# showlab/DiffSim

Measured on AMD Instinct MI355X. Metric: image-pairs/sec at 512px, SD1.5 up_blocks[0] t=600, higher is better.
Workload: dtype bf16

## Files before the change

### diffsim_amd/csrc/gemm.hip

```cpp
#include "common.h"

#include <algorithm>
#include <type_traits>

namespace dsim {

#ifdef DSIM_DEVTOOLS
int g_force_bm = 0;
int g_gemm_persistent = 1;
int g_gemm_exp = 0;
int g_gemm_skinny = 1;
unsigned long long* g_gemm_stamps = nullptr;
#endif
void gemm_tile_choice(const GemmArgs& a, int* bm, int* bn) {
    const bool geglu = a.epi == EPI_GEGLU;
    if (geglu && a.geglu_blk == 16) {
        const long tiles = (long)((a.M + 255) / 256) * (a.N / 320);
        const bool big = g_force_bm ? g_force_bm == 256 : tiles >= 256;
        *bm = big ? 256 : 128;
        *bn = big ? 320 : 160;
        return;
    }
#ifdef DSIM_DEVTOOLS
    const bool n320 = !geglu && a.N % 320 == 0 && !(g_gemm_exp & 4096), n256 = a.N % 256 == 0;
#else
    const bool n320 = !geglu && a.N % 320 == 0, n256 = a.N % 256 == 0;
#endif
    {
        const int c320 = (a.N + 319) / 320, c256 = (a.N + 255) / 256, tm = (a.M + 255) / 256, cus = cu_count();
#ifdef DSIM_DEVTOOLS
        const bool allow = !(g_gemm_exp & 16384) && !(g_gemm_exp & 4096);
#else
        const bool allow = true;
#endif
        const bool act_only = a.act == 1 && !a.gate && a.epi != EPI_RESIDUAL;
        const long r320 = ((long)tm * c320 + cus - 1) / cus, r256 = ((long)tm * c256 + cus - 1) / cus;
        if (allow && !geglu && a.mode == GEMM_LINEAR && !n320 && (act_only || (!a.act && !a.gate)) && (long)tm * c320 >= cus &&
            (long)c320 * 320 * 20 <= (long)a.N * 21 && r320 * 320 * 19 <= r256 * 256 * 20 && g_force_bm != 128) {
            *bm = 256; *bn = 320;
            return;
        }
    }
    bool n192 = !geglu && a.mode == GEMM_LINEAR && !n320 && !n256 && a.N % 192 == 0;
    if (n192 && (long)((a.N + 255) / 256) * 256 * 20 <= (long)a.N * 21 && (long)((a.M + 255) / 256) * ((a.N + 255) / 256) >= 256) {
        *bm = g_force_bm == 128 ? 128 : 256;
        *bn = g_force_bm == 128 ? 128 : 256;
        return;
    }
    const bool n128 = !geglu && a.mode == GEMM_CONV3 && a.N == 128;
    int want256 = 0;
    if (n128) {
        const long tiles = (long)((a.M + 255) / 256);
        if (tiles >= 256 && g_force_bm != 128) { *bm = 256; *bn = 128; return; }
    }
    if (n320 || n256 || n192) {
        const int bnb = n320 ? 320 : (n256 ? 256 : 192);
        const long tiles = (long)((a.M + 255) / 256) * (a.N / bnb);
        want256 = tiles >= 256;
    }
    if (a.force_big) want256 = (n320 || n256 || n192);
    if (g_force_bm == 128) want256 = 0;
    if (g_force_bm == 256) want256 = (n320 || n256 || n192);
    if (want256) { *bm = 256; *bn = n320 ? 320 : (n256 ? 256 : 192); return; }
    *bm = 128;
    *bn = (a.N % 160 == 0 && !geglu) ? 160 : 128;
#ifdef DSIM_DEVTOOLS
    const bool allow80 = !(g_gemm_exp & 2048);
#else
    const bool allow80 = true;
#endif
    if (allow80 && *bn == 160 && (long)((a.M + 127) / 128) * (a.N / 160) <= cu_count()) *bn = 80;
}

void gemm_launch_tile(const GemmArgs& a, int dtype, int* bm, int* bn) {
    gemm_tile_choice(a, bm, bn);
    const bool slow = a.act != 0 || a.gate != nullptr;
    const bool act_only = a.act == 1 && !a.gate && a.epi != EPI_RESIDUAL;
    if (*bm == 256 && *bn == 128 && dtype != DSIM_F32 && a.mode == GEMM_CONV3 && !a.bias2 && g_force_bm != 256) {
        const long hw = (long)a.Hout * a.Wout;
        if (hw >= 512L * 256 && !(hw & (hw - 1)) && a.Wout > 0 && !(a.Wout & (a.Wout - 1)) && a.M % hw == 0) *bm = 512;
    }
    if (*bm == 512) return;
    bool big = *bm == 256 && dtype != DSIM_F32;
    if (big && slow && *bn == 320 && !act_only) big = false;
    if (!big) {
        const bool n160 = *bn == 160 || (*bn == 320 && !slow) || (a.epi == EPI_GEGLU && a.geglu_blk == 16);
        const bool n80 = *bn == 80 && dtype != DSIM_F32 && !slow;
        *bm = 128;
        *bn = slow ? 128 : (n80 ? 80 : ((n160 || *bn == 80) ? 160 : 128));
    }
}

namespace {

#if defined(DSIM_DEVTOOLS) && defined(DSIM_STAMPS)
#define STAMP(t) do { __builtin_amdgcn_sched_barrier(0); asm volatile("s_memtime %0\n\ts_waitcnt lgkmcnt(0)" : "=s"(t) :: "memory"); __builtin_amdgcn_sched_barrier(0); } while (0)
#define STAMP_DECL unsigned long long st_[7] = {0, 0, 0, 0, 0, 0, 0}, sa_[6] = {0, 0, 0, 0, 0, 0}
#define STAMP_ACC(i) sa_[i] += st_[(i) + 1] - st_[i]
#else
#define STAMP(t) do { } while (0)
#define STAMP_DECL do { } while (0)
#define STAMP_ACC(i) do { } while (0)
#endif

template <typename T> struct Traits;
template <> struct Traits<h16> {
    static constexpr int BK = 64;
    static constexpr int VEC = 8;
};
template <> struct Traits<float> {
    static constexpr int BK = 32;
    static constexpr int VEC = 4;
};

template <typename T> struct Vec16T;
template <> struct Vec16T<h16> { typedef h16x8 type; };
template <> struct Vec16T<float> { typedef f32x4 type; };

__device__ __forceinline__ void load_frag(h16x8& f, const char* p) { f = *reinterpret_cast<const h16x8*>(p); }
__device__ __forceinline__ void load_frag(f32x4& f, const char* p) { f = *reinterpret_cast<const f32x4*>(p); }
__device__ __forceinline__ void mma(const h16x8& a, const h16x8& b, f32x4& c) {
    c = H16_MFMA_16x16x32(a, b, c, 0, 0, 0);
}
__device__ __forceinline__ void mma(const f32x4& a, const f32x4& b, f32x4& c) {
#pragma unroll
    for (int e = 0; e < 4; ++e) c = __builtin_amdgcn_mfma_f32_16x16x4f32(a[e], b[e], c, 0, 0, 0);
}
template <typename T> struct FragOf { typedef h16x8 type; };
template <> struct FragOf<float> { typedef f32x4 type; };

__device__ __forceinline__ float erf_as(float x) {
    const float ax = fabsf(x);
    const float t = __builtin_amdgcn_rcpf(fmaf(0.3275911f, ax, 1.0f));
    float pl = fmaf(1.061405429f, t, -1.453152027f);
    pl = fmaf(pl, t, 1.421413741f);
    pl = fmaf(pl, t, -0.284496736f);
    pl = fmaf(pl, t, 0.254829592f);
    pl *= t;
    const float e = __builtin_amdgcn_exp2f(-ax * ax * 1.4426950408889634f);
    const float r = fmaf(-pl, e, 1.0f);
    return copysignf(r, x);
}
__device__ __forceinline__ float gelu_erf(float x) { return 0.5f * x * (1.0f + erf_as(x * 0.70710678118654752f)); }

template <typename T, int BM, int BN, bool GEGLU, int WM, int WN>
constexpr int gemm_epi_bytes() {
    return WM * WN * 16 * ((GEGLU ? BN / WN / 2 : BN / WN) * (int)sizeof(T) + 16);
}
template <typename T, int BM, int BN, bool GEGLU, int WM, int WN>
constexpr int gemm_spare_bytes() {
    const int stage = (BM + BN) * 128, epi = gemm_epi_bytes<T, BM, BN, GEGLU, WM, WN>();
    return epi > stage ? ((epi - stage + 1023) / 1024) * 1024 : 0;
}
template <typename T, int BM, int BN, bool GEGLU, int WM, int WN>
constexpr int gemm_lds_bytes() {
    return 2 * (BM + BN) * 128 + gemm_spare_bytes<T, BM, BN, GEGLU, WM, WN>() +
           (BM >= 512 ? 0 : (sizeof(T) == 2 ? 2 * WM * WN * 1024 : 2 * BN * 4));
}

enum { EK_PLAIN = 0, EK_RES = 1, EK_SLOW = 2, EK_ACT = 3,
       EK_PLAIN_GN = 4, EK_RES_GN = 5 };
template <typename T, int BM, int BN, int MODE, bool GEGLU, int WM, int WN, int EKT>
__global__ __launch_bounds__(WM * WN * 64, 2) void gemm_kernel(const GemmArgs p, const int tilesN, const int ntiles, const int tilesM,
                                                               const int gn) {
    constexpr int NW = WM * WN;
    constexpr bool GNS = EKT >= EK_PLAIN_GN;
    constexpr int EK = GNS ? EKT - EK_PLAIN_GN : EKT;
    constexpr bool CONV = MODE != GEMM_LINEAR;
    constexpr bool P2 = MODE == GEMM_CONV3P;
    constexpr int BK = Traits<T>::BK;
    constexpr int VEC = Traits<T>::VEC;
    constexpr int TM = BM / (WM * 16), TN = BN / (WN * 16);
    constexpr int PS = TM >= 4 ? 2 : (TN % 5 == 0 ? 5 : 4);
    constexpr int NP = TN / PS;
    static_assert(TN % PS == 0 && (GEGLU ? TN % 2 == 0 : true), "wave tile");
    constexpr bool G16 = GEGLU && TN % 4 != 0;
    constexpr int WBN = BN / WN;
    constexpr int NA = BM / (NW * 8);
    constexpr int NBP = BN / 8;
    constexpr int NB = (NBP + NW - 1) / NW;
    constexpr int A_BYTES = BM * 128, B_BYTES = BN * 128, STAGE = A_BYTES + B_BYTES;
    constexpr int SPARE = gemm_spare_bytes<T, BM, BN, GEGLU, WM, WN>();
    typedef typename FragOf<T>::type Frag;
    extern __shared__ __attribute__((aligned(16))) char smem[];

    const int tid = threadIdx.x, lane = tid & 63, wave = tid >> 6;
    const int lrow = lane >> 3;
    const int wrow = wave * 8 + lrow;
    const unsigned celb = ((lane & 7) ^ ((wrow >> 1) & 7)) * 16;
    constexpr unsigned OOB = 0x80000000u;

    const __amdgpu_buffer_rsrc_t rA0 = __builtin_amdgcn_make_buffer_rsrc((void*)p.A0, 0, (int)p.a0_bytes, 0x00020000);
    const __amdgpu_buffer_rsrc_t rA1 = __builtin_amdgcn_make_buffer_rsrc((void*)(p.A1 ? p.A1 : p.A0), 0, (int)p.a1_bytes, 0x00020000);
    const __amdgpu_buffer_rsrc_t rW = __builtin_amdgcn_make_buffer_rsrc((void*)p.W, 0, (int)p.w_bytes, 0x00020000);
#ifdef DSIM_DEVTOOLS
    const __amdgpu_buffer_rsrc_t rO = __builtin_amdgcn_make_buffer_rsrc(p.out, 0, (p.exp & 32) ? 0 : (int)p.out_bytes, 0x00020000);
    const __amdgpu_buffer_rsrc_t rR = __builtin_amdgcn_make_buffer_rsrc((void*)(p.residual ? p.residual : p.out), 0, (p.exp & 16) ? 0 : (int)p.out_bytes, 0x00020000);
#else
    const __amdgpu_buffer_rsrc_t rO = __builtin_amdgcn_make_buffer_rsrc(p.out, 0, (int)p.out_bytes, 0x00020000);
    const __amdgpu_buffer_rsrc_t rR = __builtin_amdgcn_make_buffer_rsrc((void*)(p.residual ? p.residual : p.out), 0, (int)p.out_bytes, 0x00020000);
#endif

    int m0 = 0, n0 = 0;
    int a_iy0[NA], a_ix0[NA];
    unsigned a_base[NA], a_voff[NA];
    unsigned b_voff[NB];
    const int Hv = p.Hin << p.ups, Wv = p.Win << p.ups;
    auto setup = [&](int vb) {
        const int xcd = vb & 7, q = ntiles >> 3, r = ntiles & 7, slot = vb >> 3;
        const int bid = (xcd < r ? xcd * (q + 1) : r * (q + 1) + (xcd - r) * q) + slot;
        const int band = bid / (gn * tilesM), rem = bid - band * (gn * tilesM);
        const int bw = min(gn, tilesN - band * gn);
        const int mt = rem / bw;
        m0 = mt * BM;
        n0 = (band * gn + (rem - mt * bw)) * BN;
#pragma unroll
        for (int i = 0; i < NA; ++i) {
            const int m = m0 + i * (NW * 8) + wrow;
            if (CONV) {
                int b, oy, ox;
                if constexpr (P2) {
                    b = m >> p.lhw;
                    const int rem = m & ((1 << p.lhw) - 1);
                    oy = rem >> p.lwo; ox = rem & ((1 << p.lwo) - 1);
                } else {
                    const int hw = p.Hout * p.Wout;
                    b = m / hw;
                    const int rem = m - b * hw;
                    oy = rem / p.Wout; ox = rem - oy * p.Wout;
                }
                a_iy0[i] = (m < p.M) ? oy * p.stride - p.pad : -(1 << 20);
                a_ix0[i] = ox * p.stride - p.pad;
                a_base[i] = (unsigned)b * (unsigned)(p.Hin * p.Win);
                a_voff[i] = OOB;
            } else {
                a_iy0[i] = a_ix0[i] = 0;
                a_base[i] = (m < p.M) ? (unsigned)m : OOB;
                a_voff[i] = (m < p.M) ? (unsigned)m * (unsigned)p.C0 * (unsigned)sizeof(T) + celb : OOB;
            }
        }
        const unsigned wofs = (!CONV && p.wb_rows) ? (unsigned)(m0 / p.wb_rows) * p.wb_stride : 0u;
#pragma unroll
        for (int i = 0; i < NB; ++i) {
            const int n = n0 + i * (NW * 8) + wrow;
            b_voff[i] = (n < p.N) ? wofs + (unsigned)n * (unsigned)p.K * (unsigned)sizeof(T) + celb : OOB;
        }
    };
    const int wave_u = __builtin_amdgcn_readfirstlane(wave);
    const bool b_tail = (NBP % NW == 0) || wave_u < (NBP % NW);
    const int wm_u = wave_u / WN, wn_u = wave_u - wm_u * WN;
    constexpr bool BDMA = sizeof(T) == 2 && BM < 512;
    static_assert(!BDMA || (BN / WN) * 4 <= 1024, "bias slot");
    const __amdgpu_buffer_rsrc_t rBias = __builtin_amdgcn_make_buffer_rsrc((void*)(p.bias ? (const void*)p.bias : p.W), 0, p.bias ? p.N * 4 : 0, 0x00020000);
    auto bias_dma = [&](int par) {
        if (BDMA && !p.bias2)
            __builtin_amdgcn_raw_ptr_buffer_load_lds(rBias, (__attribute__((address_space(3))) void*)(smem + 2 * STAGE + SPARE + (par * NW + wave_u) * 1024), 16,
                                                     (int)((unsigned)(n0 + wn_u * (BN / WN)) * 4u + (unsigned)lane * 16u), 0, 0, 0);
    };

    auto derive = [&](int t) {
        const int k0 = t * BK;
        if (CONV) {
            const int tap = k0 / p.C0;
            if (k0 == tap * p.C0) {
                const int ky = tap / 3, kx = tap - ky * 3;
#pragma unroll
                for (int i = 0; i < NA; ++i) {
                    const int iy = a_iy0[i] + ky, ix = a_ix0[i] + kx;
                    const bool ok = (unsigned)iy < (unsigned)Hv && (unsigned)ix < (unsigned)Wv;
                    const unsigned pix = a_base[i] + (unsigned)((iy >> p.ups) * p.Win + (ix >> p.ups));
                    a_voff[i] = ok ? pix * (unsigned)p.C0 * (unsigned)sizeof(T) + celb : OOB;
                }
            }
        } else if (k0 == p.C0) {
#pragma unroll
            for (int i = 0; i < NA; ++i)
                a_voff[i] = a_base[i] != OOB ? a_base[i] * (unsigned)p.C1 * (unsigned)sizeof(T) + celb : OOB;
        }
    };
#define DMAW wave_u
    auto issue = [&](int t, int buf) {
        char* sa = smem + (buf ? STAGE + SPARE : 0);
        char* sb = sa + A_BYTES;
        const int k0 = t * BK;
        int soff;
        bool second = false;
        if (CONV) {
            const int tap = k0 / p.C0;
            soff = (k0 - tap * p.C0) * (int)sizeof(T);
        } else {
            second = k0 >= p.C0;
            soff = (second ? k0 - p.C0 : k0) * (int)sizeof(T);
        }
#ifdef DSIM_DEVTOOLS
        const bool skipA = CONV && (((p.exp & 64) && (k0 / p.C0) % 3 != 0) || ((p.exp & 128) && t > 0));
#else
        constexpr bool skipA = false;
#endif
        if (!skipA) {
#pragma unroll
        for (int i = 0; i < NA; ++i) {
            auto lds = (__attribute__((address_space(3))) void*)(sa + (i * NW + DMAW) * 1024);
            if (second) __builtin_amdgcn_raw_ptr_buffer_load_lds(rA1, lds, 16, (int)a_voff[i], soff, 0, 0);
            else        __builtin_amdgcn_raw_ptr_buffer_load_lds(rA0, lds, 16, (int)a_voff[i], soff, 0, 0);
        }
        }
        const int soffw = k0 * (int)sizeof(T);
#pragma unroll
        for (int i = 0; i < NB; ++i)
            if (i + 1 < NB || b_tail)
                __builtin_amdgcn_raw_ptr_buffer_load_lds(rW, (__attribute__((address_space(3))) void*)(sb + (i * NW + DMAW) * 1024),
                                                         16, (int)b_voff[i], soffw, 0, 0);
    };
    auto stage = [&](int t, int buf) { derive(t); issue(t, buf); };

    f32x4 acc[TM][TN];
    const int nk = p.K / BK;
    const int wm = wave / WN, wn = wave - wm * WN;
    const int quad = lane >> 4;
    const int foff0 = (lane & 15) * 128 + ((quad ^ ((lane >> 1) & 7)) << 4);

    Frag xf[2][TM], wf[2][PS];
    auto load_x = [&](int buf, int step, int set) {
        const char* sa = smem + (buf ? STAGE + SPARE : 0) + wm * (BM / WM) * 128 + (foff0 ^ (step << 6));
#pragma unroll
        for (int i = 0; i < TM; ++i) load_frag(xf[set][i], sa + i * 16 * 128);
    };
    auto load_w = [&](int buf, int q, int set) {
        const int step = q / NP, j0 = (q - step * NP) * PS;
        const char* sb = smem + (buf ? STAGE + SPARE : 0) + A_BYTES + (wn * WBN + j0 * 16) * 128 + (foff0 ^ (step << 6));
#pragma unroll
        for (int j = 0; j < PS; ++j) load_frag(wf[set][j], sb + j * 16 * 128);
    };
    auto mma_piece = [&](int q) {
        const int step = q / NP, j0 = (q - step * NP) * PS;
#pragma unroll
        for (int j = 0; j < PS; ++j)
#pragma unroll
            for (int i = 0; i < TM; ++i) mma(wf[q & 1][j], xf[step][i], acc[i][j0 + j]);
    };

    constexpr int ES = sizeof(T);
    constexpr int OUTW = GEGLU ? WBN / 2 : WBN;
    constexpr int RSO = OUTW * ES + 16;
    constexpr int CPR = OUTW * ES / 16;
    const int Nout = GEGLU ? (p.N >> 1) : (p.out_split ? p.out_split : p.N);
    typedef typename Vec16T<T>::type V16;
    typedef unsigned u32x4 __attribute__((ext_vector_type(4)));
    constexpr int NIT = (16 * CPR + 63) / 64;
    constexpr bool SLOW = EK == EK_SLOW;
    constexpr bool ACT = EK == EK_ACT;
    constexpr bool BIAS_INIT = !CONV || BM >= 512;
    const bool has_res = EK == EK_RES || (SLOW && p.epi == EPI_RESIDUAL);

    STAMP_DECL;
#ifdef DSIM_DEVTOOLS
    if ((p.exp >> 8) & 15) {
        if ((blockIdx.x >> 3) & 1) {
            const int n = ((p.exp >> 8) & 15) * 2;
            for (int i = 0; i < n; ++i) __builtin_amdgcn_s_sleep(127);
        }
    }
#endif
    int vb = blockIdx.x;
    int tile_par = 0;
    int b0 = 0;
    setup(vb);
    bias_dma(0);
    stage(0, 0);
    bool first = true;
    constexpr int NST = TM * NIT;
    static_assert(NST <= 60, "counted vmcnt");
    while (true) {
        STAMP(st_[0]);
        float* const bias_lds = BDMA ? reinterpret_cast<float*>(smem + 2 * STAGE + SPARE + (tile_par * NW + wave_u) * 1024) - wn_u * WBN
                                     : reinterpret_cast<float*>(smem + 2 * STAGE + SPARE) + (tile_par ? BN : 0);
        const bool bias_in_lds = !BIAS_INIT && (BDMA ? !p.bias2 : (p.bias && !p.bias2));
        if (!BDMA && bias_in_lds && tid < BN / 4) {
            const int n = n0 + tid * 4;
            f32x4 b4 = {0.f, 0.f, 0.f, 0.f};
            if (p.bias && n < p.N) b4 = *reinterpret_cast<const f32x4*>(p.bias + n);
            *reinterpret_cast<f32x4*>(bias_lds + tid * 4) = b4;
        }
        if constexpr (BDMA) {
#ifdef DSIM_DEVTOOLS
            if (first || (p.exp & 32768)) asm volatile("s_waitcnt vmcnt(0)" ::: "memory");
#else
            if (first) asm volatile("s_waitcnt vmcnt(0)" ::: "memory");
#endif
            else asm volatile("s_waitcnt vmcnt(%0)" :: "n"(NST) : "memory");
            first = false;
        }
        if (BIAS_INIT && p.bias) {
            int ilane = lane;
            asm volatile("" : "+v"(ilane));
            const int iquad = ilane >> 4, il15 = ilane & 15;
            bool odd[TM];
#pragma unroll
            for (int i = 0; i < TM; ++i)
                odd[i] = p.bias2 && (((m0 + wm * (BM / WM) + i * 16 + il15) / p.rows_per_batch) & 1);
#pragma unroll
            for (int j = 0; j < TN; ++j) {
                const int nb = n0 + wn * WBN + j * 16 + 4 * iquad;
                f32x4 b4 = {0.f, 0.f, 0.f, 0.f}, c4 = {0.f, 0.f, 0.f, 0.f};
                if (BDMA && !p.bias2) {
                    b4 = *reinterpret_cast<const f32x4*>(bias_lds + (nb - n0));
                } else if (nb < p.N) {
                    b4 = *reinterpret_cast<const f32x4*>(p.bias + nb);
                    if (p.bias2) c4 = *reinterpret_cast<const f32x4*>(p.bias2 + nb);
                }
#pragma unroll
                for (int i = 0; i < TM; ++i)
#pragma unroll
                    for (int e = 0; e < 4; ++e) acc[i][j][e] = odd[i] ? c4[e] : b4[e];
            }
        } else {
#pragma unroll
            for (int i = 0; i < TM; ++i)
#pragma unroll
                for (int j = 0; j < TN; ++j)
#pragma unroll
                    for (int r = 0; r < 4; ++r) acc[i][j][r] = 0.0f;
        }
        STAMP(st_[1]);
        if constexpr (BDMA) {
            asm volatile("s_waitcnt lgkmcnt(0)" ::: "memory");
            __builtin_amdgcn_s_barrier();
            asm volatile("" ::: "memory");
        } else {
            asm volatile("s_waitcnt vmcnt(0)" ::: "memory");
            __syncthreads();
        }
        STAMP(st_[2]);
        load_x(b0, 0, 0);
        load_w(b0, 0, 0);
        for (int t = 0; t < nk; ++t) {
            const int cur = b0 ^ (t & 1);
            if (t + 1 < nk) stage(t + 1, cur ^ 1);
#pragma unroll
            for (int q = 0; q + 1 < 2 * NP; ++q) {
                if (q == 0) load_x(cur, 1, 1);
                load_w(cur, q + 1, (q + 1) & 1);
                __builtin_amdgcn_sched_barrier(0);
                mma_piece(q);
                __builtin_amdgcn_sched_barrier(0);
            }
#ifdef DSIM_DEVTOOLS
            if (!(p.exp & 512)) asm volatile("s_waitcnt vmcnt(0)" ::: "memory");
            if (!(p.exp & 256)) __syncthreads(); else asm volatile("s_waitcnt lgkmcnt(0)" ::: "memory");
#else
            asm volatile("s_waitcnt vmcnt(0)" ::: "memory");
            __syncthreads();
#endif
            if (t + 1 < nk) { load_x(cur ^ 1, 0, 0); load_w(cur ^ 1, 0, 0); }
            __builtin_amdgcn_sched_barrier(0);
            mma_piece(2 * NP - 1);
            __builtin_amdgcn_sched_barrier(0);
        }
        STAMP(st_[3]);
        const int xbuf = b0 ^ ((nk - 1) & 1);
        const int em0 = m0, en0 = n0;
        const int nvb = vb + (int)gridDim.x;
        const bool more = nvb < ntiles;
        if (more) {
            setup(nvb);
            bias_dma(tile_par ^ 1);
            stage(0, xbuf ^ 1);
        }
        STAMP(st_[4]);
        int elane = lane;
        asm volatile("" : "+v"(elane));
        const int el15 = elane & 15, equad = elane >> 4;
        char* const wst = smem + (xbuf ? STAGE : 0) + wave * (16 * RSO);
        const int nw0 = en0 + wn * WBN;
        int osel = 0;
        if (!GEGLU && EK == EK_PLAIN && MODE == GEMM_LINEAR && p.out_split) osel = __builtin_amdgcn_readfirstlane(en0 / p.out_split);
        const __amdgpu_buffer_rsrc_t rOt = (!GEGLU && EK == EK_PLAIN && MODE == GEMM_LINEAR)
            ? __builtin_amdgcn_make_buffer_rsrc((char*)p.out + (size_t)osel * p.out_split_stride, 0, (int)p.out_bytes, 0x00020000) : rO;
        const int nout0 = (GEGLU ? (nw0 >> 1) : nw0) - osel * p.out_split;
        const int mw0 = em0 + wm * (BM / WM);
        const int mw0_u = em0 + wm_u * (BM / WM);
        const int nout0_u = (GEGLU ? ((en0 + wn_u * WBN) >> 1) : (en0 + wn_u * WBN)) - osel * p.out_split;
        const unsigned sbase = (unsigned)(mw0_u * p.ldo + nout0_u) * (unsigned)ES;
        const unsigned sslab = 16u * (unsigned)p.ldo * (unsigned)ES;
        unsigned lp[NIT];
        int lrd[NIT];
        {
            int plane = lane;
            asm volatile("" : "+v"(plane));
#pragma unroll
            for (int it = 0; it < NIT; ++it) {
                const int idx = plane + it * 64;
                const int row = idx / CPR, c = idx - row * CPR;
                lp[it] = (idx < 16 * CPR && nout0 + c * VEC < Nout) ? (unsigned)(row * p.ldo + c * VEC) * (unsigned)ES : OOB;
                lrd[it] = (row < 16 ? row : 15) * RSO + c * 16;
            }
        }
        auto piece_v = [&](int, int, int it) -> unsigned { return lp[it]; };
        auto piece_s = [&](int i) -> int { return (int)(sbase + (unsigned)i * sslab); };
        auto store_v = [&](int i, int it) -> unsigned { return lp[it] == OOB ? OOB : lp[it] + sbase + (unsigned)i * sslab; };
        constexpr int PF0 = TM > 1 ? (NIT + 1) / 2 : (NIT < 10 ? NIT : 10);
        u32x4 rres[TM][NIT];
        auto prefetch = [&](int i, int it0, int it1) {
#pragma unroll
            for (int it = 0; it < NIT; ++it)
                if (it >= it0 && it < it1)
                    rres[i][it] = __builtin_amdgcn_raw_buffer_load_b128(rR, (int)piece_v(elane, i, it), piece_s(i), 0);
        };
        constexpr bool RES16 = EK == EK_RES && sizeof(T) == 2 && !GEGLU && CONV;
        float gq[4] = {0.f, 0.f, 0.f, 0.f};
        auto gn_acc = [&](const V16& o) {
            if constexpr (GNS) {
#pragma unroll
                for (int e = 0; e < VEC; ++e) {
                    const float f = (float)o[e];
                    gq[e >> 2] += f;
                    gq[2 + (e >> 2)] = fmaf(f, f, gq[2 + (e >> 2)]);
                }
            }
        };
        if constexpr (RES16) {
            h16x4 pk[TM][TN];
            constexpr int HP = TM >= 2 ? TM / 2 : 1;
#pragma unroll
            for (int h0 = 0; h0 < TM; h0 += HP) {
                int boff = (wn * WBN + 4 * equad) * 4;
                asm volatile("" : "+v"(boff));
#pragma unroll
                for (int j = 0; j < TN; ++j) {
                    f32x4 b4 = {0.f, 0.f, 0.f, 0.f};
                    if constexpr (!BIAS_INIT) b4 = *reinterpret_cast<const f32x4*>(reinterpret_cast<const char*>(bias_lds) + boff + j * 64);
#pragma unroll
                    for (int i = h0; i < h0 + HP; ++i) {
                        typedef float f32x2 __attribute__((ext_vector_type(2)));
                        float v[4];
#pragma unroll
                        for (int e = 0; e < 4; ++e) v[e] = BIAS_INIT ? acc[i][j][e] : acc[i][j][e] + b4[e];
                        const h16x2 lo = __builtin_convertvector((f32x2){v[0], v[1]}, h16x2), hi = __builtin_convertvector((f32x2){v[2], v[3]}, h16x2);
                        pk[i][j] = (h16x4){lo[0], lo[1], hi[0], hi[1]};
                        asm volatile("" : "+v"(pk[i][j]) :: "memory");
                    }
                }
                __builtin_amdgcn_sched_barrier(0);
#pragma unroll
                for (int i = h0; i < h0 + HP; ++i) prefetch(i, 0, NIT);
                __builtin_amdgcn_sched_barrier(0);
            }
#pragma unroll
            for (int i = 0; i < TM; ++i) {
#pragma unroll
                for (int j = 0; j < TN; ++j)
                    *reinterpret_cast<h16x4*>(wst + el15 * RSO + (j * 16 + 4 * equad) * ES) = pk[i][j];
                int slane = lane;
                asm volatile("" : "+v"(slane));
#pragma unroll
                for (int it = 0; it < NIT; ++it) {
                    const V16 t = *reinterpret_cast<const V16*>(wst + lrd[it]);
                    const V16 r = __builtin_bit_cast(V16, rres[i][it]);
                    typedef float f32x2 __attribute__((ext_vector_type(2)));
                    V16 o16;
#pragma unroll
                    for (int e = 0; e < VEC; e += 2) {
                        const h16x2 pr = __builtin_convertvector((f32x2){(float)t[e] + (float)r[e], (float)t[e + 1] + (float)r[e + 1]}, h16x2);
                        o16[e] = pr[0]; o16[e + 1] = pr[1];
                    }
                    if (lp[it] != OOB) gn_acc(o16);
                    __builtin_amdgcn_raw_buffer_store_b128(__builtin_bit_cast(u32x4, o16), rO, (int)store_v(i, it), 0, 0);
                }
            }
        } else {
#pragma unroll
        for (int i = 0; i < TM; ++i) {
            __builtin_amdgcn_sched_barrier(0);
            if (has_res) prefetch(i, 0, PF0);
            __builtin_amdgcn_sched_barrier(0);
            const int slab_half_div = (SLOW && p.gate2) ? (mw0 + i * 16) / p.rows_per_batch : 0;
            const bool odd_half = !BIAS_INIT && p.bias2 && (((mw0 + i * 16 + el15) / p.rows_per_batch) & 1);
#pragma unroll
            for (int j = 0; j < TN; ++j) {
                if (GEGLU && (j & (G16 ? 1 : 2))) continue;
                float v[4];
                if (GEGLU) {
                    constexpr int JG = G16 ? 1 : 2;
#pragma unroll
                    for (int e = 0; e < 4; ++e) v[e] = acc[i][j][e] * (sizeof(T) == 2 ? gelu_fast(acc[i][j + JG][e]) : gelu_erf(acc[i][j + JG][e]));
                } else if (BIAS_INIT) {
#pragma unroll
                    for (int e = 0; e < 4; ++e) v[e] = acc[i][j][e];
                } else {
                    const int nb = nw0 + j * 16 + 4 * equad;
                    f32x4 b4 = {0.f, 0.f, 0.f, 0.f};
                    if (bias_in_lds) {
                        b4 = *reinterpret_cast<const f32x4*>(bias_lds + (nb - en0));
                    } else if (p.bias && nb < p.N) {
                        b4 = *reinterpret_cast<const f32x4*>(p.bias + nb);
                        if (p.bias2) {
                            const f32x4 c4 = *reinterpret_cast<const f32x4*>(p.bias2 + nb);
#pragma unroll
                            for (int e = 0; e < 4; ++e) b4[e] = odd_half ? c4[e] : b4[e];
                        }
                    }
#pragma unroll
                    for (int e = 0; e < 4; ++e) v[e] = acc[i][j][e] + b4[e];
                }
                const int col = (GEGLU ? (G16 ? (j >> 1) : ((j >> 2) * 2 + (j & 1))) : j) * 16 + 4 * equad;
                char* dst = wst + el15 * RSO + col * ES;
                if constexpr (sizeof(T) == 2) {
                    typedef float f32x2 __attribute__((ext_vector_type(2)));
                    const h16x2 lo = __builtin_convertvector((f32x2){v[0], v[1]}, h16x2), hi = __builtin_convertvector((f32x2){v[2], v[3]}, h16x2);
                    const h16x4 pk = {lo[0], lo[1], hi[0], hi[1]};
                    *reinterpret_cast<h16x4*>(dst) = pk;
                } else {
                    f32x4 pk = {v[0], v[1], v[2], v[3]};
                    *reinterpret_cast<f32x4*>(dst) = pk;
                }
            }
            if (has_res && PF0 < NIT) prefetch(i, PF0, NIT);
            int slane = lane;
            asm volatile("" : "+v"(slane));
#pragma unroll
            for (int it = 0; it < NIT; ++it) {
                const V16 t = *reinterpret_cast<const V16*>(wst + lrd[it]);
                if (!SLOW && !ACT && !has_res) {
                    if (lp[it] != OOB) gn_acc(t);
                    __builtin_amdgcn_raw_buffer_store_b128(__builtin_bit_cast(u32x4, t), rOt, (int)store_v(i, it), 0, 0);
                    continue;
                }
                float v[VEC];
#pragma unroll
                for (int e = 0; e < VEC; ++e) v[e] = (float)t[e];
                if (ACT || (SLOW && p.act == 1)) {
#pragma unroll
                    for (int e = 0; e < VEC; ++e) {
                        const float x = v[e];
                        const float t = x * fmaf(-0.10294324f, x * x, -2.3022082f);
                        v[e] = x * __builtin_amdgcn_rcpf(1.0f + __builtin_amdgcn_exp2f(t));
                    }
                }
                if (SLOW && p.gate) {
                    const int idx = slane + it * 64;
                    const int row = idx / CPR, c = idx - row * CPR, rrow = row < 16 ? row : 15;
                    const int m = mw0 + i * 16 + rrow, ncol = nout0 + c * VEC;
                    if (ncol < Nout) {
                        const bool odd = p.gate2 && ((((p.rows_per_batch & 15) == 0 ? slab_half_div : m / p.rows_per_batch)) & 1);
                        const float* gsel = odd ? p.gate2 : p.gate;
#pragma unroll
                        for (int e = 0; e < VEC; e += 4) {
                            const f32x4 g4 = *reinterpret_cast<const f32x4*>(gsel + ncol + e);
#pragma unroll
                            for (int f = 0; f < 4; ++f) v[e + f] *= g4[f];
                        }
                    }
                }
                if (has_res) {
                    const V16 r = __builtin_bit_cast(V16, rres[i][it]);
#pragma unroll
                    for (int e = 0; e < VEC; ++e) v[e] += (float)r[e];
                }
                V16 o16;
                if constexpr (sizeof(T) == 2) {
                    typedef float f32x2 __attribute__((ext_vector_type(2)));
#pragma unroll
                    for (int e = 0; e < VEC; e += 2) {
                        const h16x2 pr = __builtin_convertvector((f32x2){v[e], v[e + 1]}, h16x2);
                        o16[e] = pr[0]; o16[e + 1] = pr[1];
                    }
                } else {
#pragma unroll
                    for (int e = 0; e < VEC; ++e) o16[e] = (T)v[e];
                }
                __builtin_amdgcn_raw_buffer_store_b128(__builtin_bit_cast(u32x4, o16), rO, (int)store_v(i, it), 0, 0);
            }
        }
        }
        if constexpr (GNS) {
            static_assert(sizeof(T) == 2 && CONV && !GEGLU && 64 % CPR == 0 && (CPR == 8 || CPR == 16), "epilogue statistics: 64- or 128-column wave tiles");
#pragma unroll
            for (int off = 32; off >= CPR; off >>= 1)
#pragma unroll
                for (int k = 0; k < 4; ++k) gq[k] += __shfl_xor(gq[k], off, 64);
            int glane = lane;
            asm volatile("" : "+v"(glane));
            if (glane < CPR) {
                const int img = em0 / p.gn_hw, chunk = ((em0 - img * p.gn_hw) / BM) * WM + wm_u;
                const int quads = p.N >> 2, q0 = ((en0 + wn_u * WBN) >> 2) + glane * 2;
                float* o = p.gn_part + (((size_t)img * (p.gn_hw / (BM / WM)) + chunk) * quads + q0) * 2;
                *reinterpret_cast<f32x4*>(o) = (f32x4){gq[0], gq[2], gq[1], gq[3]};
            }
        }
        STAMP(st_[5]);
        STAMP_ACC(0); STAMP_ACC(1); STAMP_ACC(2); STAMP_ACC(3); STAMP_ACC(4);
        if (!more) break;
        vb = nvb;
        tile_par ^= 1;
        asm volatile("" : "+s"(vb));
        setup(vb);
        derive(0);
        b0 = xbuf ^ 1;
        STAMP(st_[6]);
        STAMP_ACC(5);
    }
#if defined(DSIM_DEVTOOLS) && defined(DSIM_STAMPS)
    if (p.stamps && lane == 0)
        for (int i = 0; i < 6; ++i) atomicAdd(p.stamps + i, sa_[i]);
    if (p.stamps && tid == 0) atomicAdd(p.stamps + 6, 1ull);
#endif
}

}

int cu_count() {
    static int per_dev[64] = {0};
    int dev = 0;
    if (hipGetDevice(&dev) != hipSuccess || dev < 0 || dev >= 64) return 256;
    int n = __atomic_load_n(&per_dev[dev], __ATOMIC_RELAXED);
    if (!n) {
        if (hipDeviceGetAttribute(&n, hipDeviceAttributeMultiprocessorCount, dev) != hipSuccess || n <= 0) n = 256;
        __atomic_store_n(&per_dev[dev], n, __ATOMIC_RELAXED);
    }
    return n;
}

int gemm_band_width(int tilesM, int tilesN, size_t w_tile_bytes) {
    (void)tilesM;
    if (tilesN <= 4) return tilesN;
    int gn = (size_t)5 * w_tile_bytes <= (size_t)2560 * 1024 ? 5 : 3;
    const int bands = (tilesN + gn - 1) / gn;
    int even = (tilesN + bands - 1) / bands;
    if (!(even & 1)) even = even > 3 ? even - 1 : 3;
    return even < gn ? even : gn;
}

int gemm_fill_extents(GemmArgs& g, size_t es) {
    size_t a0b, a1b = 16;
    if (g.mode == GEMM_CONV3) {
        const size_t bimg = (size_t)g.M / ((size_t)g.Hout * g.Wout);
        a0b = bimg * g.Hin * g.Win * g.C0 * es;
    } else {
        a0b = (size_t)g.M * g.C0 * es;
        if (g.A1) a1b = (size_t)g.M * g.C1 * es;
    }
    const size_t wb = (size_t)g.N * g.K * es + (g.wb_rows ? (size_t)(g.M / g.wb_rows - 1) * g.wb_stride : 0);
    const size_t ob = (size_t)g.M * g.ldo * es;
    if (a0b >= 0x7fffffffull || a1b >= 0x7fffffffull || wb >= 0x7fffffffull || ob >= 0x7fffffffull) return DSIM_ERR_INVALID;
    g.a0_bytes = (unsigned)a0b; g.a1_bytes = (unsigned)a1b; g.w_bytes = (unsigned)wb; g.out_bytes = (unsigned)ob;
    return DSIM_OK;
}

namespace {

template <typename T, int BM, int BN, int MODE, bool GEGLU, int WM, int WN, int EK>
int launch_ek(const GemmArgs& a, hipStream_t s) {
    constexpr int NW = WM * WN;
    constexpr int LDS = gemm_lds_bytes<T, BM, BN, GEGLU, WM, WN>();
    static_assert(LDS <= 160 * 1024, "LDS budget");
    static DeviceOnce once;
    auto kern = gemm_kernel<T, BM, BN, MODE, GEGLU, WM, WN, EK>;
    CK_ONCE(once, kern, LDS);
    const int tilesM = (a.M + BM - 1) / BM, tilesN = (a.N + BN - 1) / BN;
    GemmArgs g = a;
    const size_t es = sizeof(T);
    {
        const int st = gemm_fill_extents(g, es);
        if (st != DSIM_OK) return st;
    }
#ifdef DSIM_DEVTOOLS
    g.exp = g_gemm_exp;
    g.stamps = g_gemm_stamps;
#endif
    const int ntiles = tilesM * tilesN;
    const int resident = ((cu_count() * (LDS <= 80 * 1024 ? 2 : 1)) / 8) * 8;
    const int grid = ntiles <= resident || resident < 8 || !g_gemm_persistent ? ntiles : resident;
    int gn = gemm_band_width(tilesM, tilesN, (size_t)BN * a.K * es);
#ifdef DSIM_DEVTOOLS
    if (g_gemm_exp >> 16) gn = std::min(tilesN, g_gemm_exp >> 16);
#endif
    hipLaunchKernelGGL(kern, dim3(grid), dim3(NW * 64), LDS, s, g, tilesN, ntiles, tilesM, gn);
    DSIM_HIP_CHECK(hipGetLastError());
    return DSIM_OK;
}

template <typename T, int BM, int BN, int MODE, bool GEGLU, int WM = 4, int WN = 1, bool SLOW = false>
int launch_one(const GemmArgs& a, hipStream_t s) {
    if constexpr (SLOW) {
        if (a.act == 1 && !a.gate && a.epi != EPI_RESIDUAL) return launch_ek<T, BM, BN, MODE, GEGLU, WM, WN, EK_ACT>(a, s);
        return launch_ek<T, BM, BN, MODE, GEGLU, WM, WN, EK_SLOW>(a, s);
    }
    if constexpr (!GEGLU && sizeof(T) == 2 && MODE == GEMM_CONV3P && ((BM == 256 && (BN == 128 || BN == 256)) || (BM == 512 && BN == 128))) {
        if (a.gn_part) {
            if (a.gn_hw <= 0 || a.gn_hw % BM || a.M % a.gn_hw || a.N % BN || a.bias2) return DSIM_ERR_INVALID;
            return a.epi == EPI_RESIDUAL ? launch_ek<T, BM, BN, MODE, GEGLU, WM, WN, EK_RES_GN>(a, s)
                                         : launch_ek<T, BM, BN, MODE, GEGLU, WM, WN, EK_PLAIN_GN>(a, s);
        }
    }
    if (a.gn_part) return DSIM_ERR_INVALID;
    if constexpr (!GEGLU)
        if (a.epi == EPI_RESIDUAL) return launch_ek<T, BM, BN, MODE, GEGLU, WM, WN, EK_RES>(a, s);
    return launch_ek<T, BM, BN, MODE, GEGLU, WM, WN, EK_PLAIN>(a, s);
}

int check_args(const GemmArgs& a, int BK) {
    if (a.M <= 0 || a.N <= 0 || a.K <= 0 || a.K % BK) return DSIM_ERR_INVALID;
    if (a.mode == GEMM_CONV3) {
        if (a.C0 % BK || a.K != 9 * a.C0 || a.A1) return DSIM_ERR_INVALID;
    } else {
        if (a.C0 % BK || (a.A1 && a.C1 % BK) || a.K != a.C0 + (a.A1 ? a.C1 : 0)) return DSIM_ERR_INVALID;
    }
    if (a.epi == EPI_GEGLU && (a.mode != GEMM_LINEAR || (a.geglu_blk == 16 ? a.N % 320 != 0 : (a.geglu_blk != 32 || a.N % 64))))
        return DSIM_ERR_INVALID;
    if (!a.zero_page) return DSIM_ERR_INVALID;
    if (a.wb_rows && (a.wb_rows < 0 || a.mode != GEMM_LINEAR || a.M % a.wb_rows || a.A1 || a.epi == EPI_GEGLU || a.out_split ||
                      a.wb_stride % 16))
        return DSIM_ERR_INVALID;
    if (a.mode == GEMM_CONV3 && a.epi == EPI_RESIDUAL && a.bias2) return DSIM_ERR_INVALID;
    if (a.out_split && (a.mode != GEMM_LINEAR || a.epi != EPI_NONE || a.act || a.gate || a.out_split % 320 || a.N % a.out_split ||
                        a.out_split_stride <= 0 || (a.N / a.out_split) * a.out_split_stride >= 0x7fffffffll))
        return DSIM_ERR_INVALID;
    return DSIM_OK;
}

template <typename T>
int launch_typed(const GemmArgs& a_in, hipStream_t s) {
    const int st = check_args(a_in, Traits<T>::BK);
    if (st != DSIM_OK) return st;
    GemmArgs a = a_in;
    a.lwo = a.lhw = -1;
#ifdef DSIM_DEVTOOLS
    if (a.epi == EPI_GEGLU && (g_gemm_exp & 8192) && a.N % 64 == 0) a.geglu_blk = 32;
#endif
    if (a.mode == GEMM_CONV3) {
        const int hw = a.Hout * a.Wout;
        if (a.Wout > 0 && !(a.Wout & (a.Wout - 1)) && !(hw & (hw - 1))) {
            a.lwo = a.lhw = 0;
            while ((1 << a.lwo) < a.Wout) ++a.lwo;
            while ((1 << a.lhw) < hw) ++a.lhw;
        }
    }
    if (a.wb_rows == a.M) a.wb_rows = 0;
    if constexpr (sizeof(T) == 2) {
        if (g_gemm_skinny && !a.gn_part && !a.wb_rows && !a.force_big && gemm_skinny_applies(a)) {
            GemmArgs g = a;
            const int se = gemm_fill_extents(g, sizeof(T));
            return se != DSIM_OK ? se : launch_gemm_skinny(g, s);
        }
    }
    const bool slow = a.act != 0 || a.gate != nullptr;
    if (slow && (a.mode != GEMM_LINEAR || a.epi == EPI_GEGLU)) return DSIM_ERR_INVALID;
    int bm, bn;
    gemm_launch_tile(a, sizeof(T) == 2 ? DSIM_H16 : DSIM_F32, &bm, &bn);
    if (a.out_split && a.out_split % bn != 0) return DSIM_ERR_INVALID;
    if (a.wb_rows % bm != 0) return DSIM_ERR_INVALID;
    if constexpr (sizeof(T) == 2)
        if (bm == 512) return a.lwo >= 0 && bn == 128 ? launch_one<T, 512, 128, GEMM_CONV3P, false, 8, 1>(a, s) : DSIM_ERR_INVALID;
    const bool big = bm == 256, n160 = bn == 160;
    (void)big;
    if constexpr (sizeof(T) == 2) {
        if (big) {
            if (a.epi == EPI_GEGLU)
                return bn == 320 ? launch_one<T, 256, 320, GEMM_LINEAR, true, 4, 2>(a, s) : launch_one<T, 256, 256, GEMM_LINEAR, true, 4, 2>(a, s);
            if (a.mode == GEMM_CONV3) {
                if (bn == 128) return a.lwo >= 0 ? launch_one<T, 256, 128, GEMM_CONV3P, false, 4, 2>(a, s)
                                                 : launch_one<T, 256, 128, GEMM_CONV3, false, 4, 2>(a, s);
                if (a.lwo >= 0) return bn == 320 ? launch_one<T, 256, 320, GEMM_CONV3P, false, 4, 2>(a, s)
                                                 : launch_one<T, 256, 256, GEMM_CONV3P, false, 4, 2>(a, s);
                return bn == 320 ? launch_one<T, 256, 320, GEMM_CONV3, false, 4, 2>(a, s)
                                 : launch_one<T, 256, 256, GEMM_CONV3, false, 4, 2>(a, s);
            }
            if (slow && bn == 320) return launch_ek<T, 256, 320, GEMM_LINEAR, false, 4, 2, EK_ACT>(a, s);
            if (slow) return bn == 192 ? launch_one<T, 256, 192, GEMM_LINEAR, false, 4, 2, true>(a, s)
                                       : launch_one<T, 256, 256, GEMM_LINEAR, false, 4, 2, true>(a, s);
            if (bn == 192) return launch_one<T, 256, 192, GEMM_LINEAR, false, 4, 2>(a, s);
            return bn == 320 ? launch_one<T, 256, 320, GEMM_LINEAR, false, 4, 2>(a, s)
                             : launch_one<T, 256, 256, GEMM_LINEAR, false, 4, 2>(a, s);
        }
    }
    if (slow) return launch_one<T, 128, 128, GEMM_LINEAR, false, 4, 1, true>(a, s);
    if (a.epi == EPI_GEGLU) return n160 ? launch_one<T, 128, 160, GEMM_LINEAR, true>(a, s) : launch_one<T, 128, 128, GEMM_LINEAR, true>(a, s);
    if constexpr (sizeof(T) == 2)
        if (bn == 80) return a.mode == GEMM_CONV3 ? launch_one<T, 128, 80, GEMM_CONV3, false>(a, s) : launch_one<T, 128, 80, GEMM_LINEAR, false>(a, s);
    if (a.mode == GEMM_CONV3)
        return n160 ? launch_one<T, 128, 160, GEMM_CONV3, false>(a, s) : launch_one<T, 128, 128, GEMM_CONV3, false>(a, s);
    return n160 ? launch_one<T, 128, 160, GEMM_LINEAR, false>(a, s) : launch_one<T, 128, 128, GEMM_LINEAR, false>(a, s);
}

}

int launch_gemm(const GemmArgs& a, int dtype, hipStream_t s) {
    if (dtype == DSIM_H16) return launch_typed<h16>(a, s);
#ifndef DSIM_H16_IS_F16
    if (dtype == DSIM_F32) return launch_typed<float>(a, s);
#ifdef DSIM_HAS_F16_TWINS
    if (dtype == DSIM_F16) return launch_gemm_f16(a, dtype, s);
#endif
#endif
    return DSIM_ERR_INVALID;
}

}
```

Before: 673.1.

## Split DMA and store roles between wave halves in linear bf16 GEMM

After: 673.6 (median of 4 runs). Within noise of the previous version (+0.1%).

```diff
diff --git a/diffsim_amd/csrc/gemm.hip b/diffsim_amd/csrc/gemm.hip
--- a/diffsim_amd/csrc/gemm.hip
+++ b/diffsim_amd/csrc/gemm.hip
@@ -181,6 +181,14 @@
     constexpr int NB = (NBP + NW - 1) / NW;
     constexpr int A_BYTES = BM * 128, B_BYTES = BN * 128, STAGE = A_BYTES + B_BYTES;
     constexpr int SPARE = gemm_spare_bytes<T, BM, BN, GEGLU, WM, WN>();
+    constexpr bool SPLITK = sizeof(T) == 2 && BM == 256 && WM == 4 && WN == 2 && MODE == GEMM_LINEAR && (EK == EK_PLAIN || EK == EK_RES);
+    constexpr bool SPLITP = SPLITK && EK == EK_PLAIN && !GEGLU;
+#ifdef DSIM_DEVTOOLS
+    constexpr bool SPLITC = SPLITK;
+#else
+    constexpr bool SPLITC = SPLITP;
+#endif
+    static_assert(!SPLITC || (BN / 8) % NW == 0, "split hand-over: whole B pieces per wave");
     typedef typename FragOf<T>::type Frag;
     extern __shared__ __attribute__((aligned(16))) char smem[];
 
@@ -249,11 +257,19 @@
     const int wave_u = __builtin_amdgcn_readfirstlane(wave);
     const bool b_tail = (NBP % NW == 0) || wave_u < (NBP % NW);
     const int wm_u = wave_u / WN, wn_u = wave_u - wm_u * WN;
+#ifdef DSIM_DEVTOOLS
+    const bool split = SPLITC && ((p.exp & 2) || (SPLITP && !(p.exp & 1)));
+#else
+    constexpr bool split = SPLITP;
+#endif
+    const bool dmaw = !split || wave_u < NW / 2;
+    const float* const pbias2 = SPLITK ? nullptr : p.bias2;
+    const int bslot = dmaw ? wave_u : wave_u - NW / 2;
     constexpr bool BDMA = sizeof(T) == 2 && BM < 512;
     static_assert(!BDMA || (BN / WN) * 4 <= 1024, "bias slot");
     const __amdgpu_buffer_rsrc_t rBias = __builtin_amdgcn_make_buffer_rsrc((void*)(p.bias ? (const void*)p.bias : p.W), 0, p.bias ? p.N * 4 : 0, 0x00020000);
     auto bias_dma = [&](int par) {
-        if (BDMA && !p.bias2)
+        if (BDMA && !pbias2 && dmaw)
             __builtin_amdgcn_raw_ptr_buffer_load_lds(rBias, (__attribute__((address_space(3))) void*)(smem + 2 * STAGE + SPARE + (par * NW + wave_u) * 1024), 16,
                                                      (int)((unsigned)(n0 + wn_u * (BN / WN)) * 4u + (unsigned)lane * 16u), 0, 0, 0);
     };
@@ -280,6 +296,7 @@
     };
 #define DMAW wave_u
     auto issue = [&](int t, int buf) {
+        if (!dmaw) return;
         char* sa = smem + (buf ? STAGE + SPARE : 0);
         char* sb = sa + A_BYTES;
         const int k0 = t * BK;
@@ -305,12 +322,28 @@
             else        __builtin_amdgcn_raw_ptr_buffer_load_lds(rA0, lds, 16, (int)a_voff[i], soff, 0, 0);
         }
         }
+        if (split && !skipA) {
+            const int soff2 = soff + (NW / 2) * 8 * (second ? p.C1 : p.C0) * (int)sizeof(T);
+#pragma unroll
+            for (int i = 0; i < NA; ++i) {
+                auto lds = (__attribute__((address_space(3))) void*)(sa + (i * NW + DMAW + NW / 2) * 1024);
+                if (second) __builtin_amdgcn_raw_ptr_buffer_load_lds(rA1, lds, 16, (int)a_voff[i], soff2, 0, 0);
+                else        __builtin_amdgcn_raw_ptr_buffer_load_lds(rA0, lds, 16, (int)a_voff[i], soff2, 0, 0);
+            }
+        }
         const int soffw = k0 * (int)sizeof(T);
 #pragma unroll
         for (int i = 0; i < NB; ++i)
             if (i + 1 < NB || b_tail)
                 __builtin_amdgcn_raw_ptr_buffer_load_lds(rW, (__attribute__((address_space(3))) void*)(sb + (i * NW + DMAW) * 1024),
                                                          16, (int)b_voff[i], soffw, 0, 0);
+        if (split) {
+            const int soffw2 = soffw + (NW / 2) * 8 * p.K * (int)sizeof(T);
+#pragma unroll
+            for (int i = 0; i < NB; ++i)
+                __builtin_amdgcn_raw_ptr_buffer_load_lds(rW, (__attribute__((address_space(3))) void*)(sb + (i * NW + DMAW + NW / 2) * 1024),
+                                                         16, (int)b_voff[i], soffw2, 0, 0);
+        }
     };
     auto stage = [&](int t, int buf) { derive(t); issue(t, buf); };
 
@@ -373,7 +406,7 @@
     static_assert(NST <= 60, "counted vmcnt");
     while (true) {
         STAMP(st_[0]);
-        float* const bias_lds = BDMA ? reinterpret_cast<float*>(smem + 2 * STAGE + SPARE + (tile_par * NW + wave_u) * 1024) - wn_u * WBN
+        float* const bias_lds = BDMA ? reinterpret_cast<float*>(smem + 2 * STAGE + SPARE + (tile_par * NW + bslot) * 1024) - wn_u * WBN
                                      : reinterpret_cast<float*>(smem + 2 * STAGE + SPARE) + (tile_par ? BN : 0);
         const bool bias_in_lds = !BIAS_INIT && (BDMA ? !p.bias2 : (p.bias && !p.bias2));
         if (!BDMA && bias_in_lds && tid < BN / 4) {
@@ -383,12 +416,19 @@
             *reinterpret_cast<f32x4*>(bias_lds + tid * 4) = b4;
         }
         if constexpr (BDMA) {
-#ifdef DSIM_DEVTOOLS
-            if (first || (p.exp & 32768)) asm volatile("s_waitcnt vmcnt(0)" ::: "memory");
+            if (split) {
+                if (dmaw) asm volatile("s_waitcnt vmcnt(0)" ::: "memory");
+                asm volatile("s_waitcnt lgkmcnt(0)" ::: "memory");
+                __builtin_amdgcn_s_barrier();
+                asm volatile("" ::: "memory");
+            } else {
+#ifdef DSIM_DEVTOOLS
+                if (first || (p.exp & 32768)) asm volatile("s_waitcnt vmcnt(0)" ::: "memory");
 #else
-            if (first) asm volatile("s_waitcnt vmcnt(0)" ::: "memory");
-#endif
-            else asm volatile("s_waitcnt vmcnt(%0)" :: "n"(NST) : "memory");
+                if (first) asm volatile("s_waitcnt vmcnt(0)" ::: "memory");
+#endif
+                else asm volatile("s_waitcnt vmcnt(%0)" :: "n"(NST) : "memory");
+            }
             first = false;
         }
         if (BIAS_INIT && p.bias) {
@@ -398,16 +438,16 @@
             bool odd[TM];
 #pragma unroll
             for (int i = 0; i < TM; ++i)
-                odd[i] = p.bias2 && (((m0 + wm * (BM / WM) + i * 16 + il15) / p.rows_per_batch) & 1);
+                odd[i] = pbias2 && (((m0 + wm * (BM / WM) + i * 16 + il15) / p.rows_per_batch) & 1);
 #pragma unroll
             for (int j = 0; j < TN; ++j) {
                 const int nb = n0 + wn * WBN + j * 16 + 4 * iquad;
                 f32x4 b4 = {0.f, 0.f, 0.f, 0.f}, c4 = {0.f, 0.f, 0.f, 0.f};
-                if (BDMA && !p.bias2) {
+                if (BDMA && !pbias2) {
                     b4 = *reinterpret_cast<const f32x4*>(bias_lds + (nb - n0));
                 } else if (nb < p.N) {
                     b4 = *reinterpret_cast<const f32x4*>(p.bias + nb);
-                    if (p.bias2) c4 = *reinterpret_cast<const f32x4*>(p.bias2 + nb);
+                    if (pbias2) c4 = *reinterpret_cast<const f32x4*>(pbias2 + nb);
                 }
 #pragma unroll
                 for (int i = 0; i < TM; ++i)
@@ -424,9 +464,11 @@
         }
         STAMP(st_[1]);
         if constexpr (BDMA) {
-            asm volatile("s_waitcnt lgkmcnt(0)" ::: "memory");
-            __builtin_amdgcn_s_barrier();
-            asm volatile("" ::: "memory");
+            if (!split) {
+                asm volatile("s_waitcnt lgkmcnt(0)" ::: "memory");
+                __builtin_amdgcn_s_barrier();
+                asm volatile("" ::: "memory");
+            }
         } else {
             asm volatile("s_waitcnt vmcnt(0)" ::: "memory");
             __syncthreads();
@@ -445,6 +487,12 @@
                 mma_piece(q);
                 __builtin_amdgcn_sched_barrier(0);
             }
+            if (split) {
+                if (dmaw) asm volatile("s_waitcnt vmcnt(0)" ::: "memory");
+                asm volatile("s_waitcnt lgkmcnt(0)" ::: "memory");
+                __builtin_amdgcn_s_barrier();
+                asm volatile("" ::: "memory");
+            } else {
 #ifdef DSIM_DEVTOOLS
             if (!(p.exp & 512)) asm volatile("s_waitcnt vmcnt(0)" ::: "memory");
             if (!(p.exp & 256)) __syncthreads(); else asm volatile("s_waitcnt lgkmcnt(0)" ::: "memory");
@@ -452,6 +500,7 @@
             asm volatile("s_waitcnt vmcnt(0)" ::: "memory");
             __syncthreads();
 #endif
+            }
             if (t + 1 < nk) { load_x(cur ^ 1, 0, 0); load_w(cur ^ 1, 0, 0); }
             __builtin_amdgcn_sched_barrier(0);
             mma_piece(2 * NP - 1);
@@ -471,7 +520,10 @@
         int elane = lane;
         asm volatile("" : "+v"(elane));
         const int el15 = elane & 15, equad = elane >> 4;
-        char* const wst = smem + (xbuf ? STAGE : 0) + wave * (16 * RSO);
+        char* const ebase = smem + (xbuf ? STAGE : 0);
+        char* const wst = ebase + wave * (16 * RSO);
+        static_assert(!SPLITC || (NW + NW / 2) * 16 * RSO <= STAGE + SPARE, "split hand-over: parking slabs");
+        auto slab_buf = [&](int i) -> char* { return (split && dmaw && (i & 1)) ? ebase + (NW + wave) * (16 * RSO) : wst; };
         const int nw0 = en0 + wn * WBN;
         int osel = 0;
         if (!GEGLU && EK == EK_PLAIN && MODE == GEMM_LINEAR && p.out_split) osel = __builtin_amdgcn_readfirstlane(en0 / p.out_split);
@@ -499,6 +551,27 @@
         auto piece_v = [&](int, int, int it) -> unsigned { return lp[it]; };
         auto piece_s = [&](int i) -> int { return (int)(sbase + (unsigned)i * sslab); };
         auto store_v = [&](int i, int it) -> unsigned { return lp[it] == OOB ? OOB : lp[it] + sbase + (unsigned)i * sslab; };
+        auto handoff = [&](int i) {
+            if (!split) return;
+            asm volatile("s_waitcnt lgkmcnt(0)" ::: "memory");
+            __builtin_amdgcn_s_barrier();
+            asm volatile("" ::: "memory");
+            if (dmaw) return;
+            const unsigned sbase_p = (unsigned)((mw0_u - (WM / 2) * (BM / WM)) * p.ldo + nout0_u) * (unsigned)ES + (unsigned)i * sslab;
+            const char* pb = ebase + (((i & 1) ? NW : 0) + wave - NW / 2) * (16 * RSO);
+            int hlane = lane;
+            asm volatile("" : "+v"(hlane));
+#pragma unroll
+            for (int it = 0; it < NIT; ++it) {
+                const int idx = hlane + it * 64;
+                const V16 d = *reinterpret_cast<const V16*>(pb + (idx < 16 * CPR ? idx : 16 * CPR - 1) * 16);
+                __builtin_amdgcn_raw_buffer_store_b128(__builtin_bit_cast(u32x4, d), rOt, (int)(lp[it] == OOB ? OOB : lp[it] + sbase_p), 0, 0);
+            }
+        };
+        auto park = [&](int i, int it, const V16& o) {
+            const int idx = lane + it * 64;
+            if (idx < 16 * CPR) *reinterpret_cast<V16*>(slab_buf(i) + idx * 16) = o;
+        };
         constexpr int PF0 = TM > 1 ? (NIT + 1) / 2 : (NIT < 10 ? NIT : 10);
         u32x4 rres[TM][NIT];
         auto prefetch = [&](int i, int it0, int it1) {
@@ -604,7 +677,7 @@
                     for (int e = 0; e < 4; ++e) v[e] = acc[i][j][e] + b4[e];
                 }
                 const int col = (GEGLU ? (G16 ? (j >> 1) : ((j >> 2) * 2 + (j & 1))) : j) * 16 + 4 * equad;
-                char* dst = wst + el15 * RSO + col * ES;
+                char* dst = slab_buf(i) + el15 * RSO + col * ES;
                 if constexpr (sizeof(T) == 2) {
                     typedef float f32x2 __attribute__((ext_vector_type(2)));
                     const h16x2 lo = __builtin_convertvector((f32x2){v[0], v[1]}, h16x2), hi = __builtin_convertvector((f32x2){v[2], v[3]}, h16x2);
@@ -618,12 +691,18 @@
             if (has_res && PF0 < NIT) prefetch(i, PF0, NIT);
             int slane = lane;
             asm volatile("" : "+v"(slane));
+            V16 tall[SPLITC ? NIT : 1];
+            if constexpr (SPLITC) {
+#pragma unroll
+                for (int it = 0; it < NIT; ++it) tall[it] = *reinterpret_cast<const V16*>(slab_buf(i) + lrd[it]);
+            }
 #pragma unroll
             for (int it = 0; it < NIT; ++it) {
-                const V16 t = *reinterpret_cast<const V16*>(wst + lrd[it]);
+                const V16 t = SPLITC ? tall[SPLITC ? it : 0] : *reinterpret_cast<const V16*>(wst + lrd[it]);
                 if (!SLOW && !ACT && !has_res) {
                     if (lp[it] != OOB) gn_acc(t);
-                    __builtin_amdgcn_raw_buffer_store_b128(__builtin_bit_cast(u32x4, t), rOt, (int)store_v(i, it), 0, 0);
+                    if (split && dmaw) park(i, it, t);
+                    else __builtin_amdgcn_raw_buffer_store_b128(__builtin_bit_cast(u32x4, t), rOt, (int)store_v(i, it), 0, 0);
                     continue;
                 }
                 float v[VEC];
@@ -669,8 +748,10 @@
 #pragma unroll
                     for (int e = 0; e < VEC; ++e) o16[e] = (T)v[e];
                 }
-                __builtin_amdgcn_raw_buffer_store_b128(__builtin_bit_cast(u32x4, o16), rO, (int)store_v(i, it), 0, 0);
-            }
+                if (split && dmaw) park(i, it, o16);
+                else __builtin_amdgcn_raw_buffer_store_b128(__builtin_bit_cast(u32x4, o16), rO, (int)store_v(i, it), 0, 0);
+            }
+            handoff(i);
         }
         }
         if constexpr (GNS) {
@@ -812,7 +893,7 @@
     if (a.wb_rows && (a.wb_rows < 0 || a.mode != GEMM_LINEAR || a.M % a.wb_rows || a.A1 || a.epi == EPI_GEGLU || a.out_split ||
                       a.wb_stride % 16))
         return DSIM_ERR_INVALID;
-    if (a.mode == GEMM_CONV3 && a.epi == EPI_RESIDUAL && a.bias2) return DSIM_ERR_INVALID;
+    if (a.bias2 && (a.mode != GEMM_CONV3 || a.epi == EPI_RESIDUAL)) return DSIM_ERR_INVALID;
     if (a.out_split && (a.mode != GEMM_LINEAR || a.epi != EPI_NONE || a.act || a.gate || a.out_split % 320 || a.N % a.out_split ||
                         a.out_split_stride <= 0 || (a.N / a.out_split) * a.out_split_stride >= 0x7fffffffll))
         return DSIM_ERR_INVALID;
```
